# eikehmueller/mlmcpathintegral

Hardware: AMD Instinct MI355X
Metric: lattice-site-updates/sec (higher is better)
Workload: dtype f64

## Files before the change

mlmcpathintegral_amd/csrc/schwinger_perm.hpp:

```cpp
#pragma once
#include "lattice_sweep.hpp"

namespace mlmcpi {

#ifdef MLMCPI_STAMPS
__device__ unsigned long long g_stamps[16 * 65536];
#define MLMCPI_STAMP(k)                                                                                            \
  do {                                                                                                             \
    if (threadIdx.x == 0 && blockIdx.y * gridDim.x + blockIdx.x < 65536)                                           \
      g_stamps[(blockIdx.y * gridDim.x + blockIdx.x) * 16 + (k)] = __builtin_amdgcn_s_memrealtime();               \
  } while (0)
#define MLMCPI_STAMP_WHERE()                                                                                       \
  do {                                                                                                             \
    if (threadIdx.x == 0 && blockIdx.y * gridDim.x + blockIdx.x < 65536)                                           \
      g_stamps[(blockIdx.y * gridDim.x + blockIdx.x) * 16 + 15] =                                                  \
          ((unsigned long long)__builtin_amdgcn_s_getreg((20 ) | (0 << 6) | (31 << 11)) << 32) |         \
          __builtin_amdgcn_s_getreg((4 ) | (0 << 6) | (31 << 11));                                        \
  } while (0)
#else
#define MLMCPI_STAMP(k) do { } while (0)
#define MLMCPI_STAMP_WHERE() do { } while (0)
#endif

#ifndef MLMCPI_PERM_U
#define MLMCPI_PERM_U 0
#endif

template <class PG>
struct PermPlane {
  static constexpr int kRow = PG::kPitch * 8, kStep = kRow + 8;
  static constexpr uint32_t QB = (uint32_t)PG::kQRows * kRow;
  static_assert(kStep == (int)PG::kStep * 8, "the stride of a stream");
  uint32_t K;
  __device__ __forceinline__ explicit PermPlane(uint32_t K_) : K(K_) {}
  __device__ __forceinline__ bool has_col(uint32_t C) const { return (C & 1u) ? C <= PG::col_last(K, 1) : C >= PG::col_first(K, 0) && C <= PG::col_last(K, 0); }
  __device__ __forceinline__ bool has_row(uint32_t R) const { return (R & 1u) ? R <= PG::row_last(K, 1) : R >= PG::row_first(K, 0) && R <= PG::row_last(K, 0); }
  __device__ __forceinline__ uint32_t col(uint32_t C) const { return (C & 1u) ? QB + PG::col_u(K, C) * 8u : PG::col_u(K, C) * 8u; }
  __device__ __forceinline__ uint32_t row(uint32_t R) const { return (R & 1u) ? 2u * QB + PG::row_v(K, R) * (uint32_t)kRow : PG::row_v(K, R) * (uint32_t)kRow; }
};

struct PermBuildPos {
  uint32_t c, r, rend, row_off, gj;
  uint32_t cb;
  const double2 *src;
  uint32_t col;
  bool active, owns;
};
template <int NT, class PP>
__device__ __forceinline__ PermBuildPos perm_build_pos(const PP &P, const double2 *__restrict__ src, uint32_t Mt, uint32_t Mx, uint32_t gi0,
                                                       uint32_t gj0, uint32_t W, uint32_t rows) {
  PermBuildPos q;
  const uint32_t wave = __builtin_amdgcn_readfirstlane(threadIdx.x / kWave), lane = threadIdx.x % kWave;
  const uint32_t nwc = W > 63 ? 2 : 1;
  const uint32_t groups = (NT / kWave) >> (nwc - 1);
  const uint32_t g = wave >> (nwc - 1), cw = wave & (nwc - 1);
  static_assert(((NT / kWave) & (NT / kWave - 1)) == 0, "waves per workgroup: a power of two (shifts for divisions)");
  const uint32_t rpg = groups == 4 ? (rows + 3) >> 2 : groups == 8 ? (rows + 7) >> 3 : (rows + groups - 1) / groups;
  q.c = 63 * cw + lane;
  q.r = __builtin_amdgcn_readfirstlane(g * rpg);
  q.rend = __builtin_amdgcn_readfirstlane(g < groups ? min(rows, q.r + rpg) : 0);
  q.active = q.r < q.rend;
  q.owns = lane < 63 && q.c < W && P.has_col(q.c);
  q.cb = P.col(q.c);
  q.src = src;
  q.col = wrap_add(gi0, min(q.c, W), Mt);
  q.gj = __builtin_amdgcn_readfirstlane(wrap_add(gj0, q.r, Mx));
  q.row_off = q.gj * Mt;
  return q;
}
template <int U>
__device__ __forceinline__ void perm_rows_load(PermBuildPos &q, uint32_t Mt, uint32_t Mx, bool first, double2 &cur, double2 (&nxt)[U]) {
  if (!q.active) return;
  if (first) cur = (q.src + q.row_off)[q.col];
#pragma unroll
  for (int u = 0; u < U; ++u) {
    q.gj = q.gj + 1 == Mx ? 0 : q.gj + 1;
    q.row_off = q.gj == 0 ? 0 : q.row_off + Mt;
    if (q.r + u < q.rend) nxt[u] = (q.src + q.row_off)[q.col];
  }
}
template <int U, class PP>
__device__ __forceinline__ void perm_rows_store(PermBuildPos &q, const PP &P, double *plane, double2 &cur, const double2 (&nxt)[U]) {
  if (!q.active) return;
  char *const pb = reinterpret_cast<char *>(plane) + q.cb;
#pragma unroll
  for (int u = 0; u < U; ++u)
    if (q.r + u < q.rend) {
      const double right = wave_rotate_down(cur.y);
      if (q.owns && P.has_row(q.r + u)) *reinterpret_cast<double *>(pb + P.row(q.r + u)) = ((cur.x + right) - nxt[u].x) - cur.y;
      cur = nxt[u];
    }
  q.r += U;
}
template <int NT, int U, bool ONCE, class PP>
__device__ __forceinline__ void perm_build_rows(const PP &P, double *plane, const double2 *__restrict__ src, uint32_t Mt, uint32_t Mx,
                                                uint32_t gi0, uint32_t gj0, uint32_t W, uint32_t rows) {
  PermBuildPos q = perm_build_pos<NT>(P, src, Mt, Mx, gi0, gj0, W, rows);
  double2 cur = make_double2(0., 0.);
  if (ONCE) {
    double2 nxt[U];
    perm_rows_load<U>(q, Mt, Mx, true, cur, nxt);
    perm_rows_store<U>(q, P, plane, cur, nxt);
    return;
  }
  bool first = true;
  while (__builtin_amdgcn_readfirstlane(q.r) < __builtin_amdgcn_readfirstlane(q.rend)) {
    double2 nxt[U];
    perm_rows_load<U>(q, Mt, Mx, first, cur, nxt);
    perm_rows_store<U>(q, P, plane, cur, nxt);
    first = false;
  }
}

template <int NT, int RING, int TH = 64>
struct PermTasks {
  using PG = PermGeom<NT, RING, TH>;
  static constexpr int OW = PG::OW, HR = PG::HR, H2 = HR / 2, NW = NT / kWave, NS = (HR + NW - 1) / NW;
  static constexpr int XC = OW - 64;
  static constexpr int L0 = XC * H2, L1 = (XC / 2) * HR;
  static constexpr int NL0 = (L0 + 63) / 64, NL1 = (L1 + 63) / 64;
  static constexpr int WF = HR - NW * (NS - 1);
  static_assert(PG::NV == NS, "slots per thread");
  static_assert(NL0 + NL1 <= NW - WF, "the left-over wave-tasks fit the free last slots");
  uint32_t wave, lane, c_mu0, c_mu1, r_lo;
  __device__ PermTasks() {
    wave = __builtin_amdgcn_readfirstlane(threadIdx.x / kWave);
    lane = threadIdx.x % kWave;
    c_mu0 = lane < 32 ? 2 * lane : 2 * (lane - 32) + 1;
    c_mu1 = 2 * (lane & 31u);
    r_lo = lane >> 5;
  }
  __device__ __forceinline__ bool task(int k, bool &mu1, uint32_t &r, uint32_t &c) const {
    const uint32_t m = wave + (uint32_t)(NW * k);
    mu1 = false; r = 0; c = 0;
    if (NW * k + NW - 1 < H2 || m < (uint32_t)H2) {
      r = 2 * m;
      c = c_mu0;
      return true;
    }
    if (m < (uint32_t)HR) {
      mu1 = true;
      r = 2 * (m - H2) + r_lo;
      c = c_mu1;
      return true;
    }
    if (XC > 0 && k == NS - 1) {
      const uint32_t j = wave - (uint32_t)WF;
      if (j < (uint32_t)NL0) {
        const uint32_t L = 64 * j + lane;
        r = 2 * (L / (XC ? XC : 1));
        c = 64 + L % (XC ? XC : 1);
        return L < (uint32_t)L0;
      }
      if (j < (uint32_t)(NL0 + NL1)) {
        const uint32_t L = 64 * (j - NL0) + lane;
        mu1 = true;
        r = L / (XC > 1 ? XC / 2 : 1);
        c = 64 + 2 * (L % (XC > 1 ? XC / 2 : 1));
        return L < (uint32_t)L1;
      }
    }
    return false;
  }
  __device__ __forceinline__ bool valid(int k) const {
    bool mu1; uint32_t r, c;
    return task(k, mu1, r, c);
  }
  __device__ __forceinline__ bool is_mu1(int k) const {
    bool mu1; uint32_t r, c;
    task(k, mu1, r, c);
    return mu1;
  }
  __device__ __forceinline__ void coords(int k, uint32_t &r, uint32_t &c) const {
    bool mu1;
    task(k, mu1, r, c);
  }
};

template <int STEP>
__device__ __forceinline__ void perm_gather5(uint32_t pa, uint32_t px, uint32_t px2, double &S, double &X, double &X2) {
  double a0 = lds_read_f64<0>(pa), x0 = lds_read_f64<0>(px), y0 = lds_read_f64<0>(px2);
  double a1 = lds_read_f64<STEP>(pa), x1 = lds_read_f64<STEP>(px), y1 = lds_read_f64<STEP>(px2);
  double a2 = lds_read_f64<2 * STEP>(pa), x2 = lds_read_f64<2 * STEP>(px), y2 = lds_read_f64<2 * STEP>(px2);
  double a3 = lds_read_f64<3 * STEP>(pa), x3 = lds_read_f64<3 * STEP>(px), y3 = lds_read_f64<3 * STEP>(px2);
  double a4 = lds_read_f64<4 * STEP>(pa), x4 = lds_read_f64<4 * STEP>(px), y4 = lds_read_f64<4 * STEP>(px2);
  asm volatile("s_waitcnt lgkmcnt(0)"
               : "+v"(a0), "+v"(x0), "+v"(y0), "+v"(a1), "+v"(x1), "+v"(y1), "+v"(a2), "+v"(x2), "+v"(y2), "+v"(a3), "+v"(x3), "+v"(y3),
                 "+v"(a4), "+v"(x4), "+v"(y4)
               :
               : "memory");
  S += a0; X += x0; X2 += y0;
  S += a1; X += x1; X2 += y1;
  S += a2; X += x2; X2 += y2;
  S += a3; X += x3; X2 += y3;
  S += a4; X += x4; X2 += y4;
}
__device__ __forceinline__ void perm_gather1(uint32_t pa, uint32_t px, uint32_t px2, double &S, double &X, double &X2) {
  double a0 = lds_read_f64<0>(pa), x0 = lds_read_f64<0>(px), y0 = lds_read_f64<0>(px2);
  asm volatile("s_waitcnt lgkmcnt(0)" : "+v"(a0), "+v"(x0), "+v"(y0) : : "memory");
  S += a0; X += x0; X2 += y0;
}

template <int NT, int RING, int TH = 64>
__device__ __forceinline__ void perm_sweeps(double *plane, const double2 *__restrict__ src, uint32_t Mt, uint32_t Mx, uint32_t i0,
                                            uint32_t j0, uint32_t K, double2 (&res)[2][PermGeom<NT, RING, TH>::NV]) {
  using PG = PermGeom<NT, RING, TH>;
  using PP = PermPlane<PG>;
  constexpr int HR = PG::HR, NV = PG::NV;
  constexpr int kGroups = NT / kWave / 2;
  constexpr int U = MLMCPI_PERM_U ? MLMCPI_PERM_U : (2 * HR + 4 * (int)kPermMaxK + kGroups - 1) / kGroups;
  const uint32_t W = PG::width(K), rows = PG::rows(K), H = RING + 2 * K;
  const PP P(K);
  auto back = [](uint32_t x, uint32_t h, uint32_t n) { return h <= n ? (x >= h ? x - h : x + n - h) : (x + n - h % n) % n; };
  const uint32_t gi0 = back(i0, H, Mt), gj0 = back(j0, H, Mx);
  const uint32_t oi0 = back(i0, RING, Mt), oj0 = back(j0, RING, Mx);
  const PermTasks<NT, RING, TH> tasks;
  const char *const src_b = reinterpret_cast<const char *>(src);
  const bool small_lattice = Mx < (uint32_t)(2 * HR + 2) || Mt < (uint32_t)(PG::OW + 2);
  auto load_theta_of = [&](int h, double2 (&th)[NV], auto small) {
#pragma unroll
    for (int k = 0; k < NV; ++k) {
      if (!tasks.valid(k)) continue;
      uint32_t r, c;
      tasks.coords(k, r, c);
      uint32_t gr = oj0 + r + h * HR, gc = oi0 + c;
      gr = min(gr, gr - Mx);
      gc = min(gc, gc - Mt);
      if ((bool)small) {
        gr = min(gr, gr - Mx); gr = min(gr, gr - Mx);
        gc = min(gc, gc - Mt); gc = min(gc, gc - Mt);
      }
      const uint32_t o = (gr * Mt + gc) * 16u;
      if (!tasks.is_mu1(k)) {
        const uint32_t o2 = gr + 1 == Mx ? o - gr * Mt * 16u : o + Mt * 16u;
        th[k] = make_double2(*reinterpret_cast<const double *>(src_b + o), *reinterpret_cast<const double *>(src_b + o2));
      } else {
        const uint32_t o2 = gc + 1 == Mt ? o - gc * 16u : o + 16u;
        th[k] = make_double2(*reinterpret_cast<const double *>(src_b + o + 8u), *reinterpret_cast<const double *>(src_b + o2 + 8u));
      }
    }
  };
  auto load_theta = [&](int h, double2 (&th)[NV]) {
    if (small_lattice) load_theta_of(h, th, std::true_type{}); else load_theta_of(h, th, std::false_type{});
  };
  auto gather = [&](int h, double2 (&d)[NV]) {
    const uint32_t lds0 = (uint32_t)(uintptr_t)plane;
#pragma unroll
    for (int k = 0; k < NV; ++k) {
      if (!tasks.valid(k)) continue;
      uint32_t r, c;
      tasks.coords(k, r, c);
      const uint32_t ro = r + (uint32_t)(h * HR), cq = c >> 1, rq = ro >> 1;
      uint32_t a, x, x2;
      if (!tasks.is_mu1(k)) {
        const uint32_t cb = (c & 1u) ? PP::QB + ((uint32_t)(PG::OW / 2 - 1) - cq) * 8u : cq * 8u;
        x = cb + rq * (uint32_t)PP::kRow;
        x2 = x + (uint32_t)PP::kRow;
        a = cb + 2u * PP::QB + ((uint32_t)(HR - 1) - rq) * (uint32_t)PP::kRow;
      } else {
        const uint32_t rb = (ro & 1u) ? 2u * PP::QB + ((uint32_t)(HR - 1) - rq) * (uint32_t)PP::kRow : (rq + 1u) * (uint32_t)PP::kRow;
        x = rb + cq * 8u;
        x2 = x + 8u;
        a = rb + PP::QB + ((uint32_t)(PG::OW / 2) - cq) * 8u;
      }
      uint32_t pa = lds0 + a, px = lds0 + x, px2 = lds0 + x2;
      double S = 0.0, X = 0.0, X2 = 0.0;
      uint32_t s = 0;
      for (; s + 5 <= K; s += 5) {
        perm_gather5<PP::kStep>(pa, px, px2, S, X, X2);
        pa += 5 * PP::kStep;
        px += 5 * PP::kStep;
        px2 += 5 * PP::kStep;
      }
      for (; s < K; ++s) {
        perm_gather1(pa, px, px2, S, X, X2);
        pa += PP::kStep;
        px += PP::kStep;
        px2 += PP::kStep;
      }
      d[k] = tasks.is_mu1(k) ? make_double2(X - S, X2 - S) : make_double2(S - X, S - X2);
    }
  };
  auto finish = [&](const double2 (&th)[NV], double2 (&d)[NV]) {
#pragma unroll
    for (int k = 0; k < NV; ++k)
      if (tasks.valid(k)) d[k] = make_double2(mod_2pi_fast(th[k].x + d[k].x), mod_2pi_fast(th[k].y + d[k].y));
  };

  perm_build_rows<NT, U, MLMCPI_PERM_U == 0>(P, plane, src, Mt, Mx, gi0, gj0, W, rows);
  double2 th[NV];
  load_theta(0, th);
  __syncthreads();
  MLMCPI_STAMP(1);
  gather(0, res[0]);
  finish(th, res[0]);
  MLMCPI_STAMP(2);
  load_theta(1, th);
  gather(1, res[1]);
  finish(th, res[1]);
}

template <int NT, int RING, int TH = 64>
__device__ __forceinline__ void perm_store_image(double *th0, double *th1, const double2 (&res)[2][PermGeom<NT, RING, TH>::NV]) {
  using PG = PermGeom<NT, RING, TH>;
  constexpr int OW = PG::OW, HR = PG::HR, NV = PG::NV;
  const PermTasks<NT, RING, TH> tasks;
#pragma unroll
  for (int h = 0; h < 2; ++h)
#pragma unroll
    for (int k = 0; k < NV; ++k) {
      if (!tasks.valid(k)) continue;
      uint32_t r, c;
      tasks.coords(k, r, c);
      const uint32_t o = (r + h * HR) * OW + c;
      if (!tasks.is_mu1(k)) {
        th0[o] = res[h][k].x;
        th0[o + OW] = res[h][k].y;
      } else {
        th1[o] = res[h][k].x;
        th1[o + 1] = res[h][k].y;
      }
    }
}

}
```

Baseline: 1107 billion.

## Assign each wave a contiguous block of one kind and reuse shared row sums

Task assignment changes from interleaved waves over both mu kinds to contiguous row blocks per wave. Half the waves handle mu0 and half handle mu1, so each wave's branch is a compile-time constant. For mu0, consecutive tasks in a block share a row, so the X2 sum of one task is carried over as the X of the next, which removes one of the three LDS reads per step. This cuts LDS traffic and index arithmetic, but chains tasks serially and can unbalance the left-over work between waves.

```diff
diff --git a/mlmcpathintegral_amd/csrc/schwinger_perm.hpp b/mlmcpathintegral_amd/csrc/schwinger_perm.hpp
--- a/mlmcpathintegral_amd/csrc/schwinger_perm.hpp
+++ b/mlmcpathintegral_amd/csrc/schwinger_perm.hpp
@@ -115,65 +115,65 @@
 template <int NT, int RING, int TH = 64>
 struct PermTasks {
   using PG = PermGeom<NT, RING, TH>;
-  static constexpr int OW = PG::OW, HR = PG::HR, H2 = HR / 2, NW = NT / kWave, NS = (HR + NW - 1) / NW;
+  static constexpr int OW = PG::OW, HR = PG::HR, H2 = HR / 2, NW = NT / kWave, NS = PG::NV;
+  static constexpr int NWK = NW / 2, Q = H2 / NWK, R = H2 % NWK;
   static constexpr int XC = OW - 64;
   static constexpr int L0 = XC * H2, L1 = (XC / 2) * HR;
   static constexpr int NL0 = (L0 + 63) / 64, NL1 = (L1 + 63) / 64;
-  static constexpr int WF = HR - NW * (NS - 1);
-  static_assert(PG::NV == NS, "slots per thread");
-  static_assert(NL0 + NL1 <= NW - WF, "the left-over wave-tasks fit the free last slots");
+  static_assert(NW % 2 == 0 && NS == Q + (R > 0 ? 1 : 0), "slots per thread: the longer block");
+  static_assert(XC == 0 || (R > 0 && NL0 <= NWK - R && NL1 <= NWK - R), "the left-over wave-tasks fit the free last slots of their kind");
   uint32_t wave, lane, c_mu0, c_mu1, r_lo;
+  uint32_t j, m0, len;
+  bool kind;
   __device__ PermTasks() {
     wave = __builtin_amdgcn_readfirstlane(threadIdx.x / kWave);
     lane = threadIdx.x % kWave;
     c_mu0 = lane < 32 ? 2 * lane : 2 * (lane - 32) + 1;
     c_mu1 = 2 * (lane & 31u);
     r_lo = lane >> 5;
-  }
-  __device__ __forceinline__ bool task(int k, bool &mu1, uint32_t &r, uint32_t &c) const {
-    const uint32_t m = wave + (uint32_t)(NW * k);
-    mu1 = false; r = 0; c = 0;
-    if (NW * k + NW - 1 < H2 || m < (uint32_t)H2) {
-      r = 2 * m;
-      c = c_mu0;
-      return true;
-    }
-    if (m < (uint32_t)HR) {
-      mu1 = true;
-      r = 2 * (m - H2) + r_lo;
-      c = c_mu1;
-      return true;
-    }
-    if (XC > 0 && k == NS - 1) {
-      const uint32_t j = wave - (uint32_t)WF;
-      if (j < (uint32_t)NL0) {
-        const uint32_t L = 64 * j + lane;
+    kind = wave >= (uint32_t)NWK;
+    j = kind ? wave - (uint32_t)NWK : wave;
+    m0 = j * (uint32_t)Q + min(j, (uint32_t)R);
+    len = (uint32_t)Q + (j < (uint32_t)R ? 1u : 0u);
+  }
+  template <class F>
+  __device__ __forceinline__ void by_kind(F &&f) const {
+    if (kind) f(std::true_type{}); else f(std::false_type{});
+  }
+  __device__ __forceinline__ bool in_block(int k) const { return k < Q || (uint32_t)k < len; }
+  template <bool MU1>
+  __device__ __forceinline__ bool task(int k, uint32_t &r, uint32_t &c) const {
+    if (main_task<MU1>(k, r, c)) return true;
+    return XC > 0 && k == NS - 1 && left_task<MU1>(r, c);
+  }
+  template <bool MU1>
+  __device__ __forceinline__ bool main_task(int k, uint32_t &r, uint32_t &c) const {
+    r = 0; c = 0;
+    if (!in_block(k)) return false;
+    const uint32_t m = m0 + (uint32_t)k;
+    r = MU1 ? 2 * m + r_lo : 2 * m;
+    c = MU1 ? c_mu1 : c_mu0;
+    return true;
+  }
+  template <bool MU1>
+  __device__ __forceinline__ bool left_task(uint32_t &r, uint32_t &c) const {
+    r = 0; c = 0;
+    if (XC > 0 && !in_block(NS - 1)) {
+      const uint32_t jl = j - (uint32_t)R;
+      if (!MU1 && jl < (uint32_t)NL0) {
+        const uint32_t L = 64 * jl + lane;
         r = 2 * (L / (XC ? XC : 1));
         c = 64 + L % (XC ? XC : 1);
         return L < (uint32_t)L0;
       }
-      if (j < (uint32_t)(NL0 + NL1)) {
-        const uint32_t L = 64 * (j - NL0) + lane;
-        mu1 = true;
+      if (MU1 && jl < (uint32_t)NL1) {
+        const uint32_t L = 64 * jl + lane;
         r = L / (XC > 1 ? XC / 2 : 1);
         c = 64 + 2 * (L % (XC > 1 ? XC / 2 : 1));
         return L < (uint32_t)L1;
       }
     }
     return false;
-  }
-  __device__ __forceinline__ bool valid(int k) const {
-    bool mu1; uint32_t r, c;
-    return task(k, mu1, r, c);
-  }
-  __device__ __forceinline__ bool is_mu1(int k) const {
-    bool mu1; uint32_t r, c;
-    task(k, mu1, r, c);
-    return mu1;
-  }
-  __device__ __forceinline__ void coords(int k, uint32_t &r, uint32_t &c) const {
-    bool mu1;
-    task(k, mu1, r, c);
   }
 };
 
@@ -200,6 +200,28 @@
   asm volatile("s_waitcnt lgkmcnt(0)" : "+v"(a0), "+v"(x0), "+v"(y0) : : "memory");
   S += a0; X += x0; X2 += y0;
 }
+template <int STEP>
+__device__ __forceinline__ void perm_gather5(uint32_t pa, uint32_t px2, double &S, double &X2) {
+  double a0 = lds_read_f64<0>(pa), y0 = lds_read_f64<0>(px2);
+  double a1 = lds_read_f64<STEP>(pa), y1 = lds_read_f64<STEP>(px2);
+  double a2 = lds_read_f64<2 * STEP>(pa), y2 = lds_read_f64<2 * STEP>(px2);
+  double a3 = lds_read_f64<3 * STEP>(pa), y3 = lds_read_f64<3 * STEP>(px2);
+  double a4 = lds_read_f64<4 * STEP>(pa), y4 = lds_read_f64<4 * STEP>(px2);
+  asm volatile("s_waitcnt lgkmcnt(0)"
+               : "+v"(a0), "+v"(y0), "+v"(a1), "+v"(y1), "+v"(a2), "+v"(y2), "+v"(a3), "+v"(y3), "+v"(a4), "+v"(y4)
+               :
+               : "memory");
+  S += a0; X2 += y0;
+  S += a1; X2 += y1;
+  S += a2; X2 += y2;
+  S += a3; X2 += y3;
+  S += a4; X2 += y4;
+}
+__device__ __forceinline__ void perm_gather1(uint32_t pa, uint32_t px2, double &S, double &X2) {
+  double a0 = lds_read_f64<0>(pa), y0 = lds_read_f64<0>(px2);
+  asm volatile("s_waitcnt lgkmcnt(0)" : "+v"(a0), "+v"(y0) : : "memory");
+  S += a0; X2 += y0;
+}
 
 template <int NT, int RING, int TH = 64>
 __device__ __forceinline__ void perm_sweeps(double *plane, const double2 *__restrict__ src, uint32_t Mt, uint32_t Mx, uint32_t i0,
@@ -214,15 +236,16 @@
   auto back = [](uint32_t x, uint32_t h, uint32_t n) { return h <= n ? (x >= h ? x - h : x + n - h) : (x + n - h % n) % n; };
   const uint32_t gi0 = back(i0, H, Mt), gj0 = back(j0, H, Mx);
   const uint32_t oi0 = back(i0, RING, Mt), oj0 = back(j0, RING, Mx);
-  const PermTasks<NT, RING, TH> tasks;
+  using PT = PermTasks<NT, RING, TH>;
+  const PT tasks;
   const char *const src_b = reinterpret_cast<const char *>(src);
   const bool small_lattice = Mx < (uint32_t)(2 * HR + 2) || Mt < (uint32_t)(PG::OW + 2);
-  auto load_theta_of = [&](int h, double2 (&th)[NV], auto small) {
+  auto load_theta_of = [&](int h, double2 (&th)[NV], auto small, auto kind) {
+    constexpr bool MU1 = decltype(kind)::value;
 #pragma unroll
     for (int k = 0; k < NV; ++k) {
-      if (!tasks.valid(k)) continue;
       uint32_t r, c;
-      tasks.coords(k, r, c);
+      if (!tasks.template task<MU1>(k, r, c)) continue;
       uint32_t gr = oj0 + r + h * HR, gc = oi0 + c;
       gr = min(gr, gr - Mx);
       gc = min(gc, gc - Mt);
@@ -231,7 +254,7 @@
         gc = min(gc, gc - Mt); gc = min(gc, gc - Mt);
       }
       const uint32_t o = (gr * Mt + gc) * 16u;
-      if (!tasks.is_mu1(k)) {
+      if (!MU1) {
         const uint32_t o2 = gr + 1 == Mx ? o - gr * Mt * 16u : o + Mt * 16u;
         th[k] = make_double2(*reinterpret_cast<const double *>(src_b + o), *reinterpret_cast<const double *>(src_b + o2));
       } else {
@@ -240,19 +263,18 @@
       }
     }
   };
-  auto load_theta = [&](int h, double2 (&th)[NV]) {
-    if (small_lattice) load_theta_of(h, th, std::true_type{}); else load_theta_of(h, th, std::false_type{});
+  auto load_theta = [&](int h, double2 (&th)[NV], auto kind) {
+    if (small_lattice) load_theta_of(h, th, std::true_type{}, kind); else load_theta_of(h, th, std::false_type{}, kind);
   };
-  auto gather = [&](int h, double2 (&d)[NV]) {
+  auto gather = [&](int h, double2 (&d)[NV], auto kind) {
+    constexpr bool MU1 = decltype(kind)::value;
     const uint32_t lds0 = (uint32_t)(uintptr_t)plane;
-#pragma unroll
-    for (int k = 0; k < NV; ++k) {
-      if (!tasks.valid(k)) continue;
-      uint32_t r, c;
-      tasks.coords(k, r, c);
+    double Xnext = 0.0;
+    auto one = [&](int k, uint32_t r, uint32_t c, auto chained_t) {
+      constexpr bool chained = decltype(chained_t)::value;
       const uint32_t ro = r + (uint32_t)(h * HR), cq = c >> 1, rq = ro >> 1;
       uint32_t a, x, x2;
-      if (!tasks.is_mu1(k)) {
+      if (!MU1) {
         const uint32_t cb = (c & 1u) ? PP::QB + ((uint32_t)(PG::OW / 2 - 1) - cq) * 8u : cq * 8u;
         x = cb + rq * (uint32_t)PP::kRow;
         x2 = x + (uint32_t)PP::kRow;
@@ -266,38 +288,67 @@
       uint32_t pa = lds0 + a, px = lds0 + x, px2 = lds0 + x2;
       double S = 0.0, X = 0.0, X2 = 0.0;
       uint32_t s = 0;
-      for (; s + 5 <= K; s += 5) {
-        perm_gather5<PP::kStep>(pa, px, px2, S, X, X2);
-        pa += 5 * PP::kStep;
-        px += 5 * PP::kStep;
-        px2 += 5 * PP::kStep;
-      }
-      for (; s < K; ++s) {
-        perm_gather1(pa, px, px2, S, X, X2);
-        pa += PP::kStep;
-        px += PP::kStep;
-        px2 += PP::kStep;
-      }
-      d[k] = tasks.is_mu1(k) ? make_double2(X - S, X2 - S) : make_double2(S - X, S - X2);
+      if (chained) {
+        X = Xnext;
+        for (; s + 5 <= K; s += 5) {
+          perm_gather5<PP::kStep>(pa, px2, S, X2);
+          pa += 5 * PP::kStep;
+          px2 += 5 * PP::kStep;
+        }
+        for (; s < K; ++s) {
+          perm_gather1(pa, px2, S, X2);
+          pa += PP::kStep;
+          px2 += PP::kStep;
+        }
+      } else {
+        for (; s + 5 <= K; s += 5) {
+          perm_gather5<PP::kStep>(pa, px, px2, S, X, X2);
+          pa += 5 * PP::kStep;
+          px += 5 * PP::kStep;
+          px2 += 5 * PP::kStep;
+        }
+        for (; s < K; ++s) {
+          perm_gather1(pa, px, px2, S, X, X2);
+          pa += PP::kStep;
+          px += PP::kStep;
+          px2 += PP::kStep;
+        }
+      }
+      Xnext = X2;
+      double2 dk = MU1 ? make_double2(X - S, X2 - S) : make_double2(S - X, S - X2);
+      asm volatile("" : "+v"(dk.x), "+v"(dk.y));
+      d[k] = dk;
+    };
+    uint32_t r, c;
+    if (PT::XC > 0)
+      if (tasks.template left_task<MU1>(r, c)) one(NV - 1, r, c, std::false_type{});
+#pragma unroll
+    for (int k = 0; k < NV; ++k) {
+      if (!tasks.template main_task<MU1>(k, r, c)) continue;
+      if (!MU1 && k > 0) one(k, r, c, std::true_type{}); else one(k, r, c, std::false_type{});
     }
   };
-  auto finish = [&](const double2 (&th)[NV], double2 (&d)[NV]) {
-#pragma unroll
-    for (int k = 0; k < NV; ++k)
-      if (tasks.valid(k)) d[k] = make_double2(mod_2pi_fast(th[k].x + d[k].x), mod_2pi_fast(th[k].y + d[k].y));
+  auto finish = [&](const double2 (&th)[NV], double2 (&d)[NV], auto kind) {
+#pragma unroll
+    for (int k = 0; k < NV; ++k) {
+      uint32_t r, c;
+      if (tasks.template task<decltype(kind)::value>(k, r, c)) d[k] = make_double2(mod_2pi_fast(th[k].x + d[k].x), mod_2pi_fast(th[k].y + d[k].y));
+    }
   };
 
   perm_build_rows<NT, U, MLMCPI_PERM_U == 0>(P, plane, src, Mt, Mx, gi0, gj0, W, rows);
   double2 th[NV];
-  load_theta(0, th);
+  tasks.by_kind([&](auto kind) { load_theta(0, th, kind); });
   __syncthreads();
   MLMCPI_STAMP(1);
-  gather(0, res[0]);
-  finish(th, res[0]);
-  MLMCPI_STAMP(2);
-  load_theta(1, th);
-  gather(1, res[1]);
-  finish(th, res[1]);
+  tasks.by_kind([&](auto kind) {
+    gather(0, res[0], kind);
+    finish(th, res[0], kind);
+    MLMCPI_STAMP(2);
+    load_theta(1, th, kind);
+    gather(1, res[1], kind);
+    finish(th, res[1], kind);
+  });
 }
 
 template <int NT, int RING, int TH = 64>
@@ -305,22 +356,24 @@
   using PG = PermGeom<NT, RING, TH>;
   constexpr int OW = PG::OW, HR = PG::HR, NV = PG::NV;
   const PermTasks<NT, RING, TH> tasks;
-#pragma unroll
-  for (int h = 0; h < 2; ++h)
-#pragma unroll
-    for (int k = 0; k < NV; ++k) {
-      if (!tasks.valid(k)) continue;
-      uint32_t r, c;
-      tasks.coords(k, r, c);
-      const uint32_t o = (r + h * HR) * OW + c;
-      if (!tasks.is_mu1(k)) {
-        th0[o] = res[h][k].x;
-        th0[o + OW] = res[h][k].y;
-      } else {
-        th1[o] = res[h][k].x;
-        th1[o + 1] = res[h][k].y;
-      }
-    }
-}
-
-}
+  tasks.by_kind([&](auto kind) {
+    constexpr bool MU1 = decltype(kind)::value;
+#pragma unroll
+    for (int h = 0; h < 2; ++h)
+#pragma unroll
+      for (int k = 0; k < NV; ++k) {
+        uint32_t r, c;
+        if (!tasks.template task<MU1>(k, r, c)) continue;
+        const uint32_t o = (r + h * HR) * OW + c;
+        if (!MU1) {
+          th0[o] = res[h][k].x;
+          th0[o + OW] = res[h][k].y;
+        } else {
+          th1[o] = res[h][k].x;
+          th1[o + 1] = res[h][k].y;
+        }
+      }
+  });
+}
+
+}
```

Result: faster. 1153 billion, median of 6 (+4.1%).
